# Galtvam/OthelloZero

Hardware: AMD Instinct MI355X
Metric: mcts_node_expansions_per_sec (higher is better)
Workload: dtype f32 (3xbf16 split)

## Files before the change

include/othellozero_amd.h:

```cpp
#ifndef OTHELLOZERO_AMD_H
#define OTHELLOZERO_AMD_H
#include <stdint.h>
#ifdef __cplusplus
extern "C" {
#endif

#define OZ_OK 0
#define OZ_ERR_HIP 1
#define OZ_ERR_ARG 2
#define OZ_ERR_CAPACITY 3
#define OZ_ERR_KEY 4
#define OZ_ERR_STATE 5

#define OZ_QMODE_NEP50 0
#define OZ_QMODE_F64 1

#define OZ_LEAF_IDLE 0
#define OZ_LEAF_TERMINAL 1
#define OZ_LEAF_EVAL 2
#define OZ_LEAF_WAIT 3

const char* oz_last_error(void);
int oz_version(void);
int oz_device_count(void);
// ... 230 lines not shown
    uint64_t black, white;
    uint64_t final_black, final_white;
    uint64_t game_id;
    uint8_t ply;
    uint8_t action;
    int8_t player;
    int8_t z;
    uint8_t greedy;
    uint8_t pad[3];
} oz_record;

typedef struct {
    int64_t simulations, node_visits, expansions, terminal_hits, fallbacks;
    int64_t moves, games_completed, records;
    int32_t live_games, overflow;
    int64_t leaves_evaluated;
} oz_selfplay_stats;

int oz_selfplay_create(oz_selfplay** out, const oz_selfplay_config* cfg, oz_net* net);
int oz_selfplay_destroy(oz_selfplay* sp);
int oz_selfplay_run(oz_selfplay* sp, int rounds);
int oz_selfplay_run_steps(oz_selfplay* sp, int steps);
int oz_selfplay_set_batch_cap(oz_selfplay* sp, int cap);
int oz_selfplay_set_dedup(oz_selfplay* sp, int enable);
int oz_selfplay_set_leaves_per_step(oz_selfplay* sp, int k);
int oz_selfplay_set_solve_leaves(oz_selfplay* sp, int max_empties);
int oz_selfplay_get_solve_leaves(oz_selfplay* sp, int* max_empties, int64_t* rows_solved);
int oz_selfplay_set_value_signs(oz_selfplay* sp, int mode);
int oz_selfplay_get_value_signs(oz_selfplay* sp, int* mode);
int oz_selfplay_set_selection(oz_selfplay* sp, int flags, double fpu_reduction, double fpu_root_reduction, double cpuct_base, double cpuct_factor);
int oz_selfplay_get_selection(oz_selfplay* sp, int* flags, double* fpu_reduction, double* fpu_root_reduction, double* cpuct_base, double* cpuct_factor);
int oz_selfplay_set_proofs(oz_selfplay* sp, int enable);
int oz_selfplay_proof_stats(oz_selfplay* sp, int64_t* out4);
int oz_selfplay_solve_leaves_profile(oz_selfplay* sp, int enable);
int oz_selfplay_solve_leaves_profile_read(oz_selfplay* sp, double* ms_total, int64_t* launches, int reset);
int oz_selfplay_set_root_noise(oz_selfplay* sp, double alpha, double eps);
int oz_selfplay_root_noise(oz_selfplay* sp, double* eta, uint8_t* armed);
int oz_selfplay_set_move_sampling(oz_selfplay* sp, double temperature, int plies);
int oz_selfplay_set_playout_cap(oz_selfplay* sp, int fast_sims, double full_prob);
int oz_selfplay_get_playout_cap(oz_selfplay* sp, int* fast_sims, double* full_prob, int64_t* full_moves, int64_t* fast_moves);
int oz_selfplay_set_forced_playouts(oz_selfplay* sp, double k);
int oz_selfplay_get_forced_playouts(oz_selfplay* sp, double* k, int64_t* moves_pruned, int64_t* visits_raw, int64_t* visits_kept);
int oz_selfplay_set_resign(oz_selfplay* sp, double v, int r, int min_ply, double keep_prob);
int oz_selfplay_get_resign(oz_selfplay* sp, double* v, int* r, int* min_ply, double* keep_prob, oz_resign_stats* stats);
int oz_selfplay_sync(oz_selfplay* sp);
int oz_selfplay_stagger(oz_selfplay* sp, int sims_pre);
// ... 274 lines not shown
```

othellozero_amd/_lib.py:

```python
import ctypes as C
import os

import numpy as np

_HERE = os.path.dirname(os.path.abspath(__file__))
LIB_PATH = os.environ.get("OZ_LIB_PATH") or os.path.join(_HERE, "lib", "libothellozero_amd.so")

OZ_OK, OZ_ERR_HIP, OZ_ERR_ARG, OZ_ERR_CAPACITY, OZ_ERR_KEY, OZ_ERR_STATE = range(6)
QMODE_NEP50, QMODE_F64 = 0, 1
DEDUP_DEFAULT, DEDUP_ON, DEDUP_OFF = 0, 1, 2
NET_OPT_SIMPLE_LOOP, NET_OPT_ACT_TARGET_LOG2, NET_OPT_LOW_GUARD_LOG2, NET_OPT_SELF_CHECK, NET_OPT_W_TARGET_LOG2, NET_OPT_F32_STD_TILE, NET_OPT_LATENCY_SPLITS = 1, 2, 3, 4, 5, 6, 7
NET_OPT_CONV3_TILE = 8
NET_OPT_LOW_LOOP_PHASES = 9
NET_OPT_B3_TILE = 10
NET_OPT_B3_MIX_ROWS = 11
NET_INFO_CONV3_TILE_ROWS, NET_INFO_SELF_CHECK_GUARD, NET_INFO_ARITHMETIC = 1, 2, 3
NET_INFO_LAYER_BIG_ROWS = 64
NET_INFO_LAYER_TILE_ROWS, NET_INFO_LAYER_KSLICES, NET_INFO_LAYER_KERNEL = 16, 32, 48
NET_KERNEL_NAMES = {0: "none", 1: "f32_skinny", 2: "f32_std", 3: "f32_std_pixmajor", 4: "f32_big", 5: "lut", 6: "lut_xcd", 7: "lut_xcd_inline",
                    10: "h2_small2", 11: "h2_small", 12: "h2_bigpp", 13: "h2_bigpp_lut", 14: "h2_midpp", 15: "h2_lowpp1", 16: "h2_lowpp", 17: "h2_big",
                    18: "h2_mid", 19: "h2_thin2", 20: "h2_thin", 21: "h2_thin4w", 30: "b3", 31: "b3_big", 32: "b3_mixed"}
LEAF_IDLE, LEAF_TERMINAL, LEAF_EVAL = 0, 1, 2
VT_INT, VT_F32, VT_F64 = 0, 1, 2
MAX_LEAVES_PER_STEP = 16
# ... 221 lines not shown
    "oz_mcts_set_forced_playouts": [_vp, C.c_double], "oz_mcts_get_forced_playouts": [_vp, _f64p],
    "oz_mcts_pruned_counts": [_vp, _i32p, _u64p, _i32p],
    "oz_selfplay_set_forced_playouts": [_vp, C.c_double],
    "oz_selfplay_get_forced_playouts": [_vp, _f64p, _i64p, _i64p, _i64p],
    "oz_playout_budgets": [C.c_uint64, _u64p, _i32p, C.c_int64, C.c_int, C.c_int, C.c_double, _i32p],
    "oz_selfplay_set_resign": [_vp, C.c_double, C.c_int, C.c_int, C.c_double],
    "oz_selfplay_get_resign": [_vp, _f64p, C.POINTER(C.c_int), C.POINTER(C.c_int), _f64p, C.POINTER(ResignStats)],
    "oz_resign_scan": [_i8p, _f64p, _i32p, C.c_int64, C.c_double, C.c_int, C.c_int, _i32p, _i8p],
    "oz_resign_exempt": [C.c_uint64, _u64p, C.c_int64, C.c_double, _u8p],
    "oz_mcts_set_gumbel": [_vp, C.c_int, C.c_double, C.c_double, C.c_int, _f64p, _u8p],
    "oz_mcts_sample_gumbel": [_vp, C.c_int, C.c_double, C.c_double, C.c_int, C.c_uint64, _u64p, _i32p],
    "oz_mcts_get_gumbel": [_vp, _f64p, _u8p, _i32p, _i32p, _f64p, _f64p, _i32p],
    "oz_mcts_gumbel_policy": [_vp, _f32p, _i32p, _i32p], "oz_mcts_gumbel_scores": [_vp, _f64p],
    "oz_mcts_node_value": [_vp, C.c_int, C.c_int, _f64p],
    "oz_selfplay_set_gumbel": [_vp, C.c_int, C.c_double, C.c_double], "oz_selfplay_get_gumbel": [_vp, _i32p, _f64p, _f64p, _i64p],
    "oz_selfplay_gumbel": [_vp, _f64p, _u8p, _i32p],
    "oz_selfplay_policies": [_vp, _f32p, C.c_int64, _i64p], "oz_selfplay_policies_device": [_vp, _vp, C.c_int64, _i64p],
    "oz_gumbel_considered_visits": [C.c_int, C.c_int, _i32p],
    "oz_gumbel_draws": [C.c_uint64, _u64p, _i32p, _u64p, C.c_int64, _f64p], "oz_gumbel_from_units": [_f64p, C.c_int64, _f64p],
    "oz_gumbel_root": [_i32p, _i32p, _f64p, _f64p, _f64p, _u64p, _f64p, C.c_int64, C.c_int, C.c_double, C.c_double, C.c_int, _i32p, _i32p, _f32p,
                       _f64p, _f64p],
    "oz_selfplay_create": [C.POINTER(_vp), C.POINTER(SelfplayConfig), _vp],
    "oz_selfplay_destroy": [_vp], "oz_selfplay_run": [_vp, C.c_int], "oz_selfplay_run_steps": [_vp, C.c_int], "oz_selfplay_sync": [_vp],
    "oz_selfplay_stagger": [_vp, C.c_int], "oz_selfplay_profile": [_vp, C.c_int], "oz_selfplay_set_batch_cap": [_vp, C.c_int], "oz_selfplay_set_dedup": [_vp, C.c_int],
    "oz_selfplay_profile_read": [_vp, _f64p, _i64p, C.c_int],
    "oz_selfplay_get_stats": [_vp, C.POINTER(SelfplayStats)],
    "oz_selfplay_state": [_vp, _u64p, _u64p, _i8p, _u8p, _i32p, _u64p],
    "oz_selfplay_records": [_vp, _vp, C.c_int64, _i64p],
    "oz_selfplay_records_device": [_vp, _vp, C.c_int64, _i64p],
    "oz_selfplay_visits": [_vp, _i32p, C.c_int64, _i64p],
    "oz_selfplay_visits_device": [_vp, _vp, C.c_int64, _i64p],
    "oz_selfplay_last_counts": [_vp, _i32p],
    "oz_root_values": [_i32p, _f64p, C.c_int64, _f64p], "oz_mcts_root_values": [_vp, _f64p, _i32p],
    "oz_selfplay_set_record_values": [_vp, C.c_int],
    "oz_selfplay_values": [_vp, _f64p, C.c_int64, _i64p], "oz_selfplay_values_device": [_vp, _vp, C.c_int64, _i64p],
    "oz_selfplay_value_targets": [_vp, C.c_int64, C.c_int, C.c_double, C.c_int, C.POINTER(ValueTargetStats)],
    "oz_selfplay_targets": [_vp, _f32p, C.c_int64, _i64p], "oz_selfplay_targets_device": [_vp, _vp, C.c_int64, _i64p],
    "oz_value_targets": [_vp, _f64p, C.c_int64, C.c_int, C.c_int, C.c_double, C.c_int, _f32p],
    "oz_selfplay_set_record_surprise": [_vp, C.c_int],
    "oz_selfplay_surprises": [_vp, _f64p, C.c_int64, _i64p], "oz_selfplay_surprises_device": [_vp, _vp, C.c_int64, _i64p],
    "oz_policy_surprises": [_i32p, _f64p, C.c_int64, _f64p], "oz_policy_surprises_f32": [_f32p, _f64p, C.c_int64, _f64p],
    "oz_selfplay_surprise_weights": [_vp, C.c_int64, C.c_double, C.c_uint64, C.POINTER(SurpriseWeightStats)],
    "oz_selfplay_weights": [_vp, _f32p, _i32p, _u8p, C.c_int64, _i64p],
    "oz_surprise_weights": [_vp, _f64p, C.c_int64, C.c_double, _f32p],
    "oz_surprise_copies": [_vp, _f32p, C.c_int64, C.c_uint64, _i32p, _u8p],
    "oz_selfplay_eval_time": [_vp, _f64p, _i64p, _i64p],
    "oz_comm_unique_id": [_u8p], "oz_comm_create": [C.POINTER(_vp), _u8p, C.c_int, C.c_int], "oz_comm_destroy": [_vp],
# ... 712 lines not shown
```

othellozero_amd/csrc/oz_internal.h:

```cpp
#pragma once
#include <deque>
#include <mutex>
#include <vector>

#include "../../include/othellozero_amd.h"
#include "oz_common.h"

#define OZ_API extern "C" __attribute__((visibility("default")))

int oz_current_device();

template <auto Kernel> static int set_max_lds_once(int bytes) {
    static bool attr_done[64] = {};
    int dev_now = 0;
    OZ_HIP(hipGetDevice(&dev_now));
    if (!attr_done[dev_now & 63]) {
        OZ_HIP(hipFuncSetAttribute((const void*)Kernel, hipFuncAttributeMaxDynamicSharedMemorySize, bytes));
        attr_done[dev_now & 63] = true;
    }
    return OZ_OK;
}

struct OzTimer {
    enum { OPEN = 0, ENDED = 1, CANCELLED = 2, FAILED = 3 };
// ... 75 lines not shown
    int* d_counts = nullptr;
    EvalCacheDev ec;
    void free_eval_cache() {
        if (!ec.buckets) return;
        hipSetDevice(device);
        hipFree(ec.keys); hipFree(ec.pi); hipFree(ec.v); hipFree(ec.stamp); hipFree(ec.counters);
        ec = EvalCacheDev();
    }
    int es_mode = OZ_EVAL_SYM_OFF;
    uint64_t es_seed = 0;
    uint64_t* es_boards = nullptr;
    float* es_out = nullptr;
    int* es_count = nullptr;
    int es_profile = 0;
    OzTimer es_timer{2};
    virtual ~oz_net() {
        if (es_boards || es_out || es_count) { hipSetDevice(device); hipFree(es_boards); hipFree(es_out); hipFree(es_count); }
        es_timer.destroy();
        if (p_in) { hipSetDevice(device); hipFree(p_in); hipFree(p_out); }
        if (hp_in) { hipSetDevice(device); hipHostFree(hp_in); hipHostFree(hp_out); hipFree(d_counts); }
        free_eval_cache();
    }
    virtual int check() { return 0; }
    virtual const int* flag_device() { return nullptr; }
    virtual int forward_raw(const uint64_t* d_own, const uint64_t* d_opp, const int* d_count, int max_count,
                            float* d_pi, float* d_v, hipStream_t s) = 0;
    int forward_device(const uint64_t* d_own, const uint64_t* d_opp, const int* d_count, int max_count,
                       float* d_pi, float* d_v, hipStream_t s);
};

int oz_net_forward_device(oz_net* net, const uint64_t* d_own, const uint64_t* d_opp, const int* d_count,
                          int max_count, float* d_pi, float* d_v, hipStream_t s);

struct OzLayerShape {
    int Hin, Hout, pad, Cin, taps, N;
    int K() const { return taps * Cin; }
    int pixels() const { return Hout * Hout; }
};
template <typename Geom> inline void oz_geom_set_shape(Geom& g, const OzLayerShape& L) {
    g.Hin = L.Hin; g.Hout = L.Hout; g.pad = L.pad; g.Cin = L.Cin; g.taps = L.taps; g.N = L.N; g.K = L.K();
}
struct OzLayers {
    OzLayerShape l[5];
    const OzLayerShape& operator[](int i) const { return l[i]; }
    const OzLayerShape* begin() const { return l; }
    const OzLayerShape* end() const { return l + 5; }
// ... 47 lines not shown
```

othellozero_amd/csrc/oz_net.hip:

```cpp
#include <math.h>
#include <stdlib.h>
#include <string.h>

#include <algorithm>
#include <type_traits>
#include <vector>

#include "oz_internal.h"

__global__ __launch_bounds__(256) void k_conv1(const uint64_t* __restrict__ own, const uint64_t* __restrict__ opp,
                                               const int* __restrict__ d_count, int n, int C,
                                               const float* __restrict__ W , const float* __restrict__ scale,
                                               const float* __restrict__ shift, float* __restrict__ out ) {
    const int P = n * n, cq = C >> 2;
    const long long M = (long long)(*d_count) * P;
    const long long idx = (long long)blockIdx.x * blockDim.x + threadIdx.x;
    const long long m = idx / cq;
    if (m >= M) return;
    const int c4 = (int)(idx % cq) * 4;
    const int b = (int)(m / P), pix = (int)(m % P), y = pix / n, x = pix % n;
    const uint64_t o = own[b], p = opp[b];
    float acc0 = 0.f, acc1 = 0.f, acc2 = 0.f, acc3 = 0.f;
#pragma unroll
    for (int ky = 0; ky < 3; ++ky)
// ... 816 lines not shown
    float *d_scale1_h2 = nullptr, *d_shift1_h2 = nullptr;
    float* d_shift_h2[5] = {nullptr, nullptr, nullptr, nullptr, nullptr};
    unsigned* d_lowcnt[5] = {nullptr, nullptr, nullptr, nullptr, nullptr};
    unsigned char* d_lut_low = nullptr;
    unsigned fwd_seq = 0;
    int act_target_log2 = H2_ACT_TOP;
    int w_target_log2 = H2_W_TOP;
    int low_guard_log2 = H2_LOW_GUARD;
    float low_thr = 0.f;
    int self_check = 1;
    double sc_dpi = -1.0, sc_dv = -1.0;
    int sc_positions = 0;
    int sc_guard = 0;
    float *d_sc_out = nullptr;
    uint64_t *d_cal_own = nullptr, *d_cal_opp = nullptr;
    int* d_cal_count = nullptr;
    int cal_total = 0;

    uint4* d_wb[5] = {nullptr, nullptr, nullptr, nullptr, nullptr};
    uint4* b3a1 = nullptr;
    uint4 *b3a2 = nullptr, *b3a3 = nullptr, *b3a4 = nullptr, *b3f1 = nullptr;
    float* d_part_b3 = nullptr;
    bool use_b3() const { return precision == 2 && max_batch >= B3_MIN_BATCH; }
    int fc1_b3_ksplit() const {
        const long long blocks = (((long long)max_batch + B3_BM - 1) / B3_BM) * 4;
        int k = 1;
        while (k < 8 && blocks * k < 192) k *= 2;
        return k < 2 ? 2 : k;
    }
    int conv_b3_ksplit(int pixels) const {
        const long long blocks = (((long long)max_batch * pixels + B3_BM - 1) / B3_BM) * (C / B3_BN);
        int k = 1;
        while (k < 8 && blocks * k < 192) k *= 2;
        return k;
    }
    int ensure_b3a1() {
        if (b3a1 || !use_b3() || (tables_mode != 0 && tables_mode != 1)) return OZ_OK;
        return alloc(&b3a1, (size_t)max_batch * n * n * (C / 32 * 12));
    }
    int fc2_b3_ksplit() const {
        return 4;
    }

    struct TimedSlot {
        OzTimer* t = nullptr;
        hipStream_t s;
// ... 1166 lines not shown
    OnnNet* o = as_onn(net);
    OZ_REQUIRE(o && out, "not an OthelloNN network / null argument");
    OZ_REQUIRE(which >= 0 && which <= 9, "oz_net_get_scaling: which must be 0 .. 9 (got %d)", which);
    std::lock_guard<std::mutex> lk(o->mu);
    OZ_REQUIRE(o->precision == 1 && o->committed, "oz_net_get_scaling: the network is not committed in precision f16x2");
    const std::vector<int>& e = which < 5 ? o->aexp[which] : o->wexp[which - 5];
    OZ_REQUIRE(nelem == (int64_t)e.size(), "oz_net_get_scaling(%d): %lld elements expected, got %lld", which, (long long)e.size(), (long long)nelem);
    for (size_t i = 0; i < e.size(); ++i) out[i] = e[i];
    return OZ_OK;
}

OZ_API int oz_net_get_info(oz_net* net, int what, int* value) {
    OnnNet* o = as_onn(net);
    OZ_REQUIRE(o && value, "not an OthelloNN network / null argument");
    std::lock_guard<std::mutex> lk(o->mu);
    for (int l = 1; l <= 5; ++l) {
        const OnnNet::LayerPlan& p = o->plan[l];
        if (what == OZ_NET_INFO_LAYER_TILE_ROWS(l)) { *value = p.tile_rows; return OZ_OK; }
        if (what == OZ_NET_INFO_LAYER_KSLICES(l)) { *value = p.ksplit; return OZ_OK; }
        if (what == OZ_NET_INFO_LAYER_KERNEL(l)) { *value = p.kernel; return OZ_OK; }
        if (what == OZ_NET_INFO_LAYER_BIG_ROWS(l)) { *value = (int)p.big_rows; return OZ_OK; }
    }
    OZ_REQUIRE(what == OZ_NET_INFO_CONV3_TILE_ROWS || what == OZ_NET_INFO_SELF_CHECK_GUARD || what == OZ_NET_INFO_ARITHMETIC, "unknown network info %d", what);
    *value = what == OZ_NET_INFO_CONV3_TILE_ROWS ? o->last_conv3_rows : what == OZ_NET_INFO_ARITHMETIC ? (o->precision == 2 && !o->use_b3() ? 0 : o->precision) : o->sc_guard;
    return OZ_OK;
}

OZ_API int oz_net_b3_plan(int n, int channels, int max_batch, int layer, int kslices, int tile_opt, int mix_rows_opt, int* kernel, int64_t* big_rows,
                          int64_t* small_tiles) {
    OZ_REQUIRE((n == 6 || n == 8) && channels > 0 && channels % B3_BN == 0 && max_batch >= 1 && layer >= 1 && layer <= 5 && kslices >= 1,
               "oz_net_b3_plan: bad shape (n=%d channels=%d max_batch=%d layer=%d kslices=%d)", n, channels, max_batch, layer, kslices);
    OZ_REQUIRE(tile_opt == 0 || tile_opt == 128 || tile_opt == 256, "OZ_NET_OPT_B3_TILE must be 0, 128 or 256 (got %d)", tile_opt);
    OZ_REQUIRE(mix_rows_opt <= 0 || mix_rows_opt % B3B_BM == 0, "OZ_NET_OPT_B3_MIX_ROWS must be 0, negative or a positive multiple of 256 (got %d)", mix_rows_opt);
    const OzLayerShape L = oz_onn_layers(n, channels)[layer - 1];
    const long long rows_cap = (long long)max_batch * L.pixels();
    const long long head = b3_plan_rows(L, rows_cap, kslices, tile_opt, mix_rows_opt);
    const int k = b3_plan_kernel(head, rows_cap);
    if (kernel) *kernel = k;
    if (big_rows) *big_rows = k == OZ_NET_KERNEL_B3 ? 0 : head;
    if (small_tiles) *small_tiles = k == OZ_NET_KERNEL_B3_BIG ? 0 : (rows_cap + B3_BM - 1) / B3_BM - (k == OZ_NET_KERNEL_B3 ? 0 : head / B3_BM);
    return OZ_OK;
}

OZ_API int oz_net_get_activation(oz_net* net, int layer, int64_t first_row, int64_t rows, double* out) {
    OnnNet* o = as_onn(net);
    OZ_REQUIRE(o && out, "oz_net_get_activation: not an OthelloNN network / null argument");
    OZ_REQUIRE(layer >= 0 && layer <= 5, "oz_net_get_activation: layer must be 0 .. 5 (got %d)", layer);
// ... 61 lines not shown
```

othellozero_amd/csrc/oz_search.hip:

```cpp
#pragma clang fp contract(off)
#include <math.h>
#include <string.h>

#include "oz_internal.h"
#include "oz_minimax.h"
#include "oz_openings.h"
#include "oz_solve.h"

enum { VT_INT = 0, VT_F32 = 1, VT_F64 = 2 };
#define OZ_MAX_DEPTH 64
#define OZ_TAG_F32 0x80000000u
#define OZ_NSTAT 5
enum { ST_SIMS = 0, ST_VISITS = 1, ST_EXPAND = 2, ST_TERMINAL = 3, ST_FALLBACK = 4 };
enum { EF_NODES = 1, EF_EDGES = 2, EF_DEPTH = 4, EF_NOMOVE = 8, EF_RECORDS = 16, EF_ROOT = 32, EF_CORRUPT = 64 };

struct OzEdge { uint32_t n_tag; int32_t child; double q; double p; };
#define OZ_REC_HDR 32
#define OZ_EDGE_BYTES 24
#define OZ_HT_IDX_BITS 20
#define OZ_HT_IDX_MASK ((1u << OZ_HT_IDX_BITS) - 1u)
static_assert(sizeof(OzEdge) == OZ_EDGE_BYTES, "edge layout");

enum { PS_EDGES = 0, PS_EDGE_STOPS = 1, PS_NODE_STOPS = 2, PS_ROOTS = 3, OZ_NPSTAT = 4 };
struct ProofDev {
// ... 443 lines not shown
    if (!t.active[g]) {
        if (lane == 0) t.leaf_status[g] = OZ_LEAF_IDLE;
        return OZ_LEAF_IDLE;
    }
    double eta = 0.0;
    const bool noisy = noise_of_slot<NOISE>(t, g, lane, &eta);
    const uint64_t own = uni64(t.root_own[g]), opp = uni64(t.root_opp[g]);
    int rootn = unii(t.root_node[g]);
    GumbelRoot gr{false, 0.0, 0, nullptr};
    if constexpr (GUMBEL) gr = gumbel_of_slot(*gd, g, lane);
    const Descent e = descend_one<NOISE, GUMBEL, VS, SEL>(t, L.rec, L.path, g, lane, own, opp, oz_legal(own, opp, t.valid), rootn, noisy, eta, InFlight{nullptr, nullptr, 0}, gr);
    __syncthreads();
    if (lane < e.depth) t.path[(size_t)g * OZ_MAX_DEPTH + lane] = L.path[lane];
    if (lane == 0) {
        t.leaf_status[g] = e.status;
        t.leaf_own[g] = e.own; t.leaf_opp[g] = e.opp; t.leaf_legal[g] = e.legal; t.leaf_fs[g] = e.fs;
        t.depth[g] = e.depth; t.term_value[g] = e.tval;
        unsigned long long* st = t.stat + (size_t)g * OZ_NSTAT;
        st[ST_SIMS] += 1; st[ST_VISITS] += (unsigned long long)(e.depth + 1);
        if (e.status == OZ_LEAF_TERMINAL) st[ST_TERMINAL] += 1;
        if (e.err) atomicOr(t.error_flag, e.err);
    }
    return e.status;
}

__device__ __forceinline__ unsigned ec_bucket(const EvalCacheDev& c, uint64_t own, uint64_t opp, unsigned* way_pick) {
    const uint64_t h = key_hash64(own ^ 0x6A09E667F3BCC909ULL, opp);
    *way_pick = (unsigned)(h >> 40) & (OZ_EC_WAYS - 1);
    return (unsigned)(h >> 8) & (c.buckets - 1);
}
__device__ __forceinline__ int ec_find(const EvalCacheDev& c, uint64_t own, uint64_t opp) {
    unsigned pick;
    const unsigned b = ec_bucket(c, own, opp, &pick);
    const ulonglong2* k = reinterpret_cast<const ulonglong2*>(c.keys) + (size_t)b * OZ_EC_WAYS;
#pragma unroll
    for (int w = 0; w < OZ_EC_WAYS; ++w) {
        const ulonglong2 e = k[w];
        if (e.x == own && e.y == opp) return (int)(b * OZ_EC_WAYS + w);
    }
    return -1;
}
__global__ __launch_bounds__(256) void k_cache_copy(MctsDev t) {
    const int idx = blockIdx.x * 256 + threadIdx.x, h = idx >> 6, a = idx & 63;
    if (h >= *t.hit_count) return;
    const int e = t.hit_entry[h], row = t.G - 1 - h;
    if (a < t.n2) t.pi[(size_t)row * t.n2 + a] = t.ec.pi[(size_t)e * t.n2 + a];
// ... 2764 lines not shown
    } else if (lane == 0) {
        gm.black[g] = black; gm.white[g] = white; gm.player[g] = (int8_t)player;
        gm.finished[g] = (uint8_t)fin; gm.ply[g] = nply;
        t.root_node[g] = -1;
    }
}
enum : unsigned { MV_SAMPLE = 1, MV_CAP = 2, MV_FORCE = 4, MV_VALUES = 8, MV_GUMBEL = 16, MV_SURPRISE = 32, MV_RESIGN = 64, MV_PROVEN = 128,
                  MV_FULL = MV_SAMPLE | MV_CAP | MV_FORCE | MV_VALUES };
struct MoveArgs {
    MoveSampling ms; PlayoutCap pc; ForcedPlayouts fp; SurprisePlay su; ResignPlay rs; ProofPlay pp; GumbelPlay gp;
    int arena;
};
template <unsigned M>
__global__ __launch_bounds__(64) void k_sp_move(GamesDev gm, MctsDev t, MoveArgs a) {
    const int arena = M == 0 ? a.arena : M == MV_PROVEN ? 1 : 0;
    sp_move_body<false, has(M, MV_SAMPLE), has(M, MV_CAP), has(M, MV_FORCE), has(M, MV_VALUES), has(M, MV_GUMBEL), has(M, MV_SURPRISE), has(M, MV_RESIGN),
                 has(M, MV_PROVEN)>(gm, t, blockIdx.x, threadIdx.x, arena, a.ms, a.pc, a.fp, a.gp, a.su, a.rs, a.pp);
}

#define OZ_ADVANCE_CAP 2
struct SelfplayExtras { double alpha; uint64_t seed; MoveSampling sample; PlayoutCap cap; ForcedPlayouts forced; };
template <bool EXTRAS = false, bool VALUES = EXTRAS, bool SURPRISE = false, int VS = OZ_VSIGNS_REFERENCE>
__device__ __forceinline__ void advance_body(const GamesDev& gm, const MctsDev& t, TreeLds& L, int g, int lane, int sims, int* __restrict__ sims_done, int cap,
                                             SelfplayExtras xt = SelfplayExtras{}, SurprisePlay su = SurprisePlay{}) {
    if (unii(t.leaf_status[g]) == OZ_LEAF_WAIT) {
        if (lane == 0) t.leaf_status[g] = OZ_LEAF_EVAL;
        return;
    }
    int done = sims_done[g];
    if (t.leaf_status[g] == OZ_LEAF_EVAL) ++done;
    int status = OZ_LEAF_IDLE;
    for (int it = 0; it < cap; ++it) {
        if (gm.finished[g]) { if (lane == 0) { t.active[g] = 0; t.leaf_status[g] = OZ_LEAF_IDLE; } status = OZ_LEAF_IDLE; break; }
        const int p = gm.player[g];
        if (lane == 0) {
            t.active[g] = 1;
            t.root_own[g] = p == 1 ? gm.black[g] : gm.white[g];
            t.root_opp[g] = p == 1 ? gm.white[g] : gm.black[g];
        }
        wave_sync();
        int budget = sims, fast = 0;
        if constexpr (EXTRAS) {
            if (xt.cap.fast_sims > 0)
                budget = oz_playout_budget(gm.seed, uni64(gm.game_id[g]), (uint64_t)unii(gm.ply[g]), sims, xt.cap.fast_sims, xt.cap.full_prob, &fast);
        }
        if (done >= budget) {
            sp_move_body<EXTRAS, EXTRAS, EXTRAS, EXTRAS, VALUES, false, SURPRISE>(gm, t, g, lane, 0, xt.sample, xt.cap, xt.forced, GumbelPlay{}, su);
            done = 0;
            if (lane == 0) t.leaf_status[g] = OZ_LEAF_IDLE;
            wave_sync();
            continue;
        }
        if constexpr (EXTRAS) {
            if (t.noise_eps > 0.0 && !fast && unii((int)t.noise_armed[g]) == 0) {
                root_noise_body(t, L.arr, g, lane, uni64(t.root_own[g]), uni64(t.root_opp[g]), xt.alpha, xt.seed, uni64(gm.game_id[g]), unii(gm.ply[g]));
                wave_sync();
            }
        }
        status = select_body<EXTRAS, false, VS>(t, L, g, lane);
        if (status != OZ_LEAF_TERMINAL) break;
        wave_sync();
        backup_body<VS>(t, g, lane, (double)t.term_value[g], VT_INT);
        ++done;
        status = OZ_LEAF_IDLE;
        if (lane == 0) t.leaf_status[g] = OZ_LEAF_IDLE;
        wave_sync();
    }
    if (lane == 0) sims_done[g] = done;
}
enum : unsigned { AV_SIGNS = 3, AV_EXTRAS = 4, AV_VALUES = 8, AV_SURPRISE = 16 };
struct AdvanceArgs { SelfplayExtras xt; SurprisePlay su; };
template <unsigned A>
__global__ __launch_bounds__(64) void k_advance(GamesDev gm, MctsDev t, int sims, int* __restrict__ sims_done, int cap, AdvanceArgs a) {
    __shared__ TreeLds L;
    advance_body<has(A, AV_EXTRAS), has(A, AV_VALUES), has(A, AV_SURPRISE), int(A & AV_SIGNS)>(gm, t, L, blockIdx.x, threadIdx.x, sims, sims_done, cap, a.xt, a.su);
}
template <unsigned A>
__global__ __launch_bounds__(64) void k_backup_advance(GamesDev gm, MctsDev t, int sims, int* __restrict__ sims_done, int cap, AdvanceArgs a) {
    __shared__ TreeLds L;
    expand_backup_body<false, int(A & AV_SIGNS)>(t, L, blockIdx.x, threadIdx.x, 0);
    backup_fence();
    advance_body<has(A, AV_EXTRAS), has(A, AV_VALUES), has(A, AV_SURPRISE), int(A & AV_SIGNS)>(gm, t, L, blockIdx.x, threadIdx.x, sims, sims_done, cap, a.xt, a.su);
}

__global__ void k_arena_random_move(GamesDev gm, int side) {
    const int g = blockIdx.x * blockDim.x + threadIdx.x;
    if (g >= gm.G || gm.finished[g] || gm.player[g] != side) return;
    uint64_t black = gm.black[g], white = gm.white[g];
    int player = side, fin = 0;
    const uint64_t legal = oz_legal(side == 1 ? black : white, side == 1 ? white : black, gm.valid);
    const int ply = gm.ply[g];
    const int action = oz_kth_bit(legal, (int)(oz_rng(gm.seed, gm.game_id[g], (uint64_t)ply, OZ_RNG_TIE) % (uint64_t)oz_popc(legal)));
    const size_t lb = (size_t)g * 64;
    if (ply < 64) {
        gm.log_black[lb + ply] = black; gm.log_white[lb + ply] = white;
        gm.log_action[lb + ply] = (uint8_t)action; gm.log_player[lb + ply] = (int8_t)player; gm.log_greedy[lb + ply] = 0;
    }
    oz_game_play(black, white, player, fin, action, gm.valid);
    gm.black[g] = black; gm.white[g] = white; gm.player[g] = (int8_t)player;
    gm.finished[g] = (uint8_t)fin; gm.ply[g] = ply + 1;
    atomicAdd(&gm.counters[2], 1ULL);
}

__global__ __launch_bounds__(64) void k_arena_minimax_move(GamesDev gm, int side, int depth, MinimaxEval ev) {
    __shared__ MinimaxLds L;
// ... 25 lines not shown
    const int played = oz_opening_play(gm.n, gm.valid, op.moves ? op.n_plies[g] : op.plies, op.moves ? op.moves + (size_t)g * OZ_OPENING_MAX_PLIES : nullptr,
                                       op.seed, op.first_id + (uint64_t)g, black, white, player, fin,
                                       [&](int ply, uint64_t b, uint64_t w, int p, int action) {
                                           gm.log_black[lb + ply] = b; gm.log_white[lb + ply] = w;
                                           gm.log_action[lb + ply] = (uint8_t)action; gm.log_player[lb + ply] = (int8_t)p; gm.log_greedy[lb + ply] = 0;
                                       });
    gm.black[g] = black; gm.white[g] = white; gm.player[g] = (int8_t)player;
    gm.finished[g] = (uint8_t)fin; gm.ply[g] = played;
    op.opening_plies[g] = played;
    if (played) atomicAdd(&gm.counters[2], (unsigned long long)played);
}

static void initial_board(int n, uint64_t* black, uint64_t* white) { oz_initial_board(n, *black, *white); }

struct oz_selfplay {
    oz_selfplay_config cfg;
    oz_mcts* m = nullptr;
    oz_net* net = nullptr;
    GamesDev gm;
    int* d_sims_done = nullptr;
    int mode = 0;
    int batch_cap = 0;
    long long batch_no = 0;
    int stagger_period = 0;
    bool noise_on = false;
    double noise_alpha = 0.0;
    MoveSampling sample{0.0, 0};
    PlayoutCap cap{0, 0.0, nullptr, nullptr};
    ForcedPlayouts forced{0.0, nullptr};
    bool gumbel_on = false;
    float *gumbel_log = nullptr, *gumbel_rows = nullptr;
    unsigned long long* gumbel_moves = nullptr;
    std::vector<void*> allocs;
    std::mutex mu;
    long long records_read = 0;
    long long* d_endgame = nullptr;
    double *val_log = nullptr, *val_rec = nullptr;
    float* targets = nullptr;
    long long* d_vt = nullptr;
    double *sur_log = nullptr, *sur_rec = nullptr;
    SurprisePlay su{nullptr, nullptr};
    float* weights = nullptr;
    int32_t* copies = nullptr;
    uint8_t* first_sym = nullptr;
    long long* d_sw = nullptr;
    ResignPlay resign{0.0, 0.0, 0, 0, nullptr, nullptr, nullptr, nullptr, nullptr};
// ... 619 lines not shown
    if (moves && sp->gumbel_moves) {
        hipSetDevice(sp->m->device);
        OZ_HIP(hipStreamSynchronize(sp->m->stream));
        OZ_HIP(hipMemcpy(&c, sp->gumbel_moves, sizeof c, hipMemcpyDeviceToHost));
    }
    if (moves) *moves = (int64_t)c;
    return OZ_OK;
}
OZ_API int oz_selfplay_gumbel(oz_selfplay* sp, double* g, uint8_t* armed, int32_t* N0) {
    OZ_REQUIRE(sp, "null selfplay");
    { std::lock_guard<std::mutex> lk(sp->mu); hipSetDevice(sp->m->device); OZ_HIP(hipStreamSynchronize(sp->m->stream)); }
    return oz_mcts_get_gumbel(sp->m, g, armed, N0, nullptr, nullptr, nullptr, nullptr);
}
OZ_API int oz_selfplay_root_noise(oz_selfplay* sp, double* eta, uint8_t* armed) {
    OZ_REQUIRE(sp, "null selfplay");
    std::lock_guard<std::mutex> lk(sp->mu);
    std::lock_guard<std::mutex> lkm(sp->m->mu);
    hipSetDevice(sp->m->device);
    OZ_HIP(hipStreamSynchronize(sp->m->stream));
    return noise_read_locked(sp->m, eta, armed);
}

struct AdvanceKernels {
    void (*advance)(GamesDev, MctsDev, int, int*, int, AdvanceArgs);
    void (*backup_advance)(GamesDev, MctsDev, int, int*, int, AdvanceArgs);
    void (*expand_backup)(MctsDev, int);
};
static int advance_kernels(const oz_selfplay* sp, AdvanceKernels* k, AdvanceArgs* a) {
    const oz_mcts* m = sp->m;
    const bool surprise = sp->su.log != nullptr;
    const bool extras = surprise || m->noise_ever || sp->sample.plies > 0 || sp->cap.fast_sims > 0;
    *a = AdvanceArgs{};
    if (extras) a->xt = SelfplayExtras{sp->noise_alpha, sp->gm.seed, sp->sample, sp->cap, sp->forced};
    if (surprise) a->su = sp->su;
    const unsigned signs = m->proofs ? OZ_VSIGNS_PROVEN : m->vsigns != OZ_VSIGNS_REFERENCE ? OZ_VSIGNS_SOUND : OZ_VSIGNS_REFERENCE;
    const unsigned v = signs | (extras ? AV_EXTRAS : 0) | (extras || sp->gm.log_values ? AV_VALUES : 0) | (surprise ? AV_SURPRISE : 0);
    switch (v) {
#define OZ_A(...) \
    case (__VA_ARGS__): *k = AdvanceKernels{k_advance<(__VA_ARGS__)>, k_backup_advance<(__VA_ARGS__)>, k_expand_backup<(__VA_ARGS__) & AV_SIGNS>}; return OZ_OK
        OZ_A(OZ_VSIGNS_REFERENCE); OZ_A(OZ_VSIGNS_REFERENCE | AV_VALUES); OZ_A(OZ_VSIGNS_REFERENCE | AV_EXTRAS | AV_VALUES);
        OZ_A(OZ_VSIGNS_REFERENCE | AV_EXTRAS | AV_VALUES | AV_SURPRISE);
        OZ_A(OZ_VSIGNS_SOUND); OZ_A(OZ_VSIGNS_SOUND | AV_VALUES); OZ_A(OZ_VSIGNS_SOUND | AV_EXTRAS | AV_VALUES);
        OZ_A(OZ_VSIGNS_SOUND | AV_EXTRAS | AV_VALUES | AV_SURPRISE);
#undef OZ_A
    }
    oz_set_error("oz_selfplay_run_steps: the free-running driver has no kernels for this combination of options (variant 0x%x); use oz_selfplay_run", v);
    return OZ_ERR_STATE;
}
// ... 1 lines not shown
OZ_API int oz_selfplay_run_steps(oz_selfplay* sp, int steps) {
    OZ_REQUIRE(sp, "null selfplay");
    std::lock_guard<std::mutex> lk(sp->mu);
    if (sp->m->leaves_per_step > 1) {
        oz_set_error("oz_selfplay_run_steps: the free-running driver runs one leaf per game and batch (leaves_per_step is %d); use oz_selfplay_run", sp->m->leaves_per_step);
        return OZ_ERR_STATE;
    }
    if (sp->gumbel_on) { oz_set_error("oz_selfplay_run_steps: the free-running driver does not run the Gumbel search; use oz_selfplay_run"); return OZ_ERR_STATE; }
    if (sp->m->proofs) { oz_set_error("oz_selfplay_run_steps: the free-running driver keeps no proofs; use oz_selfplay_run"); return OZ_ERR_STATE; }
    if (sp->m->d.sel.flags) { oz_set_error("oz_selfplay_run_steps: the free-running kernels have no selection instantiation; use oz_selfplay_run"); return OZ_ERR_STATE; }
    if (sp->resign.r > 0) { oz_set_error("oz_selfplay_run_steps: the free-running driver does not resign games; use oz_selfplay_run"); return OZ_ERR_STATE; }
    if (sp->tree_gc != OZ_TREE_GC_OFF) { oz_set_error("oz_selfplay_run_steps: the free-running driver moves inside its kernels and does not collect the tree; use oz_selfplay_run"); return OZ_ERR_STATE; }
    std::lock_guard<std::mutex> lkn(sp->net->mu);
    oz_mcts* m = sp->m;
    hipSetDevice(m->device);
    MctsDev& d = m->d;
    if (sp->mode == 1) OZ_HIP(hipMemsetAsync(d.leaf_status, 0, sizeof(int) * d.G, m->stream));
    if (sp->mode == 1 && m->noise_ever) OZ_HIP(hipMemsetAsync(d.noise_armed, 0, (size_t)d.G, m->stream));
    sp->mode = 2;
    selfplay_attach_cache(sp);
    AdvanceKernels ak;
    AdvanceArgs aargs;
    if (int rc = advance_kernels(sp, &ak, &aargs)) return rc;
    for (int i = 0; i < steps; ++i) {
        const bool all = m->profile;
        hipStream_t s = m->stream;
        const int adv_cap = (sp->batch_cap > 0 && sp->batch_cap < d.G ? 1 : OZ_ADVANCE_CAP);
        timed(m, TS_SELECT, all, [&] { hipLaunchKernelGGL(i == 0 ? ak.advance : ak.backup_advance, dim3(d.G), dim3(64), 0, s, sp->gm, d, sp->cfg.sims, sp->d_sims_done, adv_cap, aargs); });
        MctsDev dc = d;
        const int cap = sp->batch_cap > 0 && sp->batch_cap < d.G ? sp->batch_cap : 0;
        dc.batch_cap = cap;
        dc.batch_rot = cap ? (int)((sp->batch_no * (long long)cap) % d.G) : 0;
        sp->batch_no += 1;
        timed(m, TS_COMPACT, all, [&] { hipLaunchKernelGGL(k_compact, dim3(1), dim3(1024), 0, s, dc); });
        if (int rc = eval_batch_async(m, sp->net, cap ? cap : d.G, true)) return rc;
        if (i == steps - 1) timed(m, TS_BACKUP, all, [&] { hipLaunchKernelGGL(ak.expand_backup, dim3(d.G), dim3(64), 0, s, d, 0); });
        OZ_HIP(hipGetLastError());
        if (m->timer.backlog() > 4096) m->timer.drain();
    }
    return OZ_OK;
}

OZ_API int oz_selfplay_set_batch_cap(oz_selfplay* sp, int cap) {
    OZ_REQUIRE(sp, "null selfplay");
    std::lock_guard<std::mutex> lk(sp->mu);
    OZ_REQUIRE(cap >= 0, "oz_selfplay_set_batch_cap: cap %d", cap);
    OZ_REQUIRE(cap == 0 || cap >= 8, "oz_selfplay_set_batch_cap: a cap below 8 leaves (got %d)", cap);
    sp->batch_cap = cap;
    return OZ_OK;
}

OZ_API int oz_selfplay_set_dedup(oz_selfplay* sp, int enable) {
    OZ_REQUIRE(sp, "null selfplay");
    std::lock_guard<std::mutex> lk(sp->mu);
    sp->m->d.dedup = enable ? 1 : 0;
    return OZ_OK;
}

OZ_API int oz_selfplay_sync(oz_selfplay* sp) {
    OZ_REQUIRE(sp, "null selfplay");
    std::lock_guard<std::mutex> lk(sp->mu);
    hipSetDevice(sp->m->device);
// ... 1378 lines not shown
```

othellozero_amd/training.py:

```python
import ctypes as C
import logging
import random

import numpy as np

from . import _lib
from .NNet import NeuralNets
from .Othello import BoardView, OthelloGame, OthelloPlayer
from .othelo_mcts import OthelloMCTS


def training_example_symmetries(board, policy):
    symetric_examples = []
    for rotation in range(1, 5):
        for flip in (True, False):
            b, p = np.rot90(board, k=rotation), np.rot90(policy, k=rotation)
            if flip:
                b, p = np.fliplr(b), np.fliplr(p)
            symetric_examples.append((b, p))
    return symetric_examples


def execute_episode(board_size, neural_network, degree_exploration, num_simulations, policy_temperature, e_greedy,
                    q_mode=_lib.QMODE_F64, snapshot_boards=False, policy_target="onehot", target_temperature=1.0,
# ... 281 lines not shown
        return rows.value

    def __del__(self):
        try:
            if self._h:
                _lib.load().oz_selfplay_destroy(self._h)
                self._h = C.c_void_p()
        except Exception:
            pass

    def run(self, rounds=1, sync=True):
        _lib.check(_lib.load().oz_selfplay_run(self._h, int(rounds)))
        if sync:
            self.sync()

    def run_steps(self, steps, sync=True):
        _lib.check(_lib.load().oz_selfplay_run_steps(self._h, int(steps)))
        if sync:
            self.sync()

    def set_batch_cap(self, cap):
        _lib.check(_lib.load().oz_selfplay_set_batch_cap(self._h, int(cap)))

    def set_dedup(self, enable):
        _lib.check(_lib.load().oz_selfplay_set_dedup(self._h, 1 if enable else 0))

    def stagger(self, sims_pre=None, sync=True):
        _lib.check(_lib.load().oz_selfplay_stagger(self._h, int(sims_pre or self.cfg.sims)))
        if sync:
            self.sync()

    def profile(self, enable=True):
        _lib.check(_lib.load().oz_selfplay_profile(self._h, 1 if enable else 0))

    def profile_read(self, reset=False):
        k = len(_lib.TREE_KERNELS)
        ms, cnt = np.zeros(k, np.float64), np.zeros(k, np.int64)
        _lib.check(_lib.load().oz_selfplay_profile_read(self._h, _lib.p_f64(ms), _lib.p_i64(cnt), 1 if reset else 0))
        return {name: (float(ms[i]), int(cnt[i])) for i, name in enumerate(_lib.TREE_KERNELS)}

    def sync(self):
        _lib.check(_lib.load().oz_selfplay_sync(self._h))

    def stats(self):
        s = _lib.SelfplayStats()
        _lib.check(_lib.load().oz_selfplay_get_stats(self._h, C.byref(s)))
# ... 91 lines not shown
        return written.value

    def eval_time(self):
        ms, launches, leaves = C.c_double(), C.c_int64(), C.c_int64()
        _lib.check(_lib.load().oz_selfplay_eval_time(self._h, C.byref(ms), C.byref(launches), C.byref(leaves)))
        return dict(ms=ms.value, launches=launches.value, leaves=leaves.value)

    def play_to_end(self, max_rounds=None, with_visits=False, endgame_targets=0, value_target="outcome", with_policies=False,
                    proof_targets=False):
        proof_targets = _lib.check_proof_targets(proof_targets, self.proof_play)
        max_rounds = max_rounds or self.n * self.n
        for _ in range(max_rounds):
            self.run(4)
            if self.stats()["live_games"] == 0:
                break
        if proof_targets:
            self.proof_target_stats = self.proof_targets()
        if endgame_targets:
            self.endgame_stats = self.solve_records(endgame_targets)
        if _lib.check_value_target(value_target)[0] != _lib.VALUE_TARGET_OUTCOME:
            self.value_target_stats = self.value_targets(value_target, exact_empties=endgame_targets, exact_proven=proof_targets)
            return self.records(with_visits=with_visits, with_targets=True, with_policies=with_policies)
        return self.records(with_visits=with_visits, with_policies=with_policies)


def preferred_batch_cap(board_size, num_games, channels=512, precision="f16x2"):
    if channels % 256 or num_games < 1024 or precision == "bf16x3":
        return 0
    P, cols = (board_size - 2) ** 2, channels // 256
    rounds = (num_games * P // 256) * cols // 256
    if rounds < 1:
        return 0
    cap = (256 * rounds // cols) * 256 // P
    return 0 if cap >= num_games else int(cap)


def expand_examples(records, board_size, alias_final=False, visits=None, target_temperature=1.0, values=None):
    if values is not None:
        rec_all = np.ascontiguousarray(records, dtype=_lib.RECORD_DTYPE)
        val = np.ascontiguousarray(values, dtype=np.float32).ravel()
        assert val.size == rec_all.size, f"{val.size} value targets for {rec_all.size} records"
        boards, pol, _z = expand_examples(rec_all, board_size, alias_final, visits=visits, target_temperature=target_temperature)
        return boards, pol, np.repeat(val[_lib.record_fast(rec_all).ravel() == 0], 8)
    records, visits = _lib.full_records(np.ascontiguousarray(records, dtype=_lib.RECORD_DTYPE), visits)
    rec = np.ascontiguousarray(records, dtype=_lib.RECORD_DTYPE)
    R, n = rec.size, board_size
# ... 124 lines not shown
```

Measured before the change: 960,200.

## Restructure advance kernel to cache root state and batch stat updates

The per-game advance kernel now loads the root position, its legal-move mask and the root node once per move rather than on every loop iteration. It calls descend_one directly and stores the descent result to global memory only when a leaf actually needs evaluation. Per-simulation statistics are accumulated in registers and written once at the end, and a separate cap for idle entry is added along with a setter and a defaults API. Default caps are unchanged, so the gain is meant to come from fewer global memory writes and reloads in the select/terminal-backup loop, at the cost of more complex control flow.

New measurement: 959,900 (median of 2 runs). Within noise of the previous version (-0.0%).

```diff
diff --git a/include/othellozero_amd.h b/include/othellozero_amd.h
--- a/include/othellozero_amd.h
+++ b/include/othellozero_amd.h
@@ -276,6 +276,8 @@
 int oz_selfplay_run(oz_selfplay* sp, int rounds);
 int oz_selfplay_run_steps(oz_selfplay* sp, int steps);
 int oz_selfplay_set_batch_cap(oz_selfplay* sp, int cap);
+int oz_selfplay_set_advance_cap(oz_selfplay* sp, int cap, int cap_idle);
+int oz_selfplay_advance_caps(int arithmetic, int games, int batch_cap, int* cap, int* cap_idle);
 int oz_selfplay_set_dedup(oz_selfplay* sp, int enable);
 int oz_selfplay_set_leaves_per_step(oz_selfplay* sp, int k);
 int oz_selfplay_set_solve_leaves(oz_selfplay* sp, int max_empties);
diff --git a/othellozero_amd/_lib.py b/othellozero_amd/_lib.py
--- a/othellozero_amd/_lib.py
+++ b/othellozero_amd/_lib.py
@@ -267,7 +267,9 @@
                        _f64p, _f64p],
     "oz_selfplay_create": [C.POINTER(_vp), C.POINTER(SelfplayConfig), _vp],
     "oz_selfplay_destroy": [_vp], "oz_selfplay_run": [_vp, C.c_int], "oz_selfplay_run_steps": [_vp, C.c_int], "oz_selfplay_sync": [_vp],
-    "oz_selfplay_stagger": [_vp, C.c_int], "oz_selfplay_profile": [_vp, C.c_int], "oz_selfplay_set_batch_cap": [_vp, C.c_int], "oz_selfplay_set_dedup": [_vp, C.c_int],
+    "oz_selfplay_stagger": [_vp, C.c_int], "oz_selfplay_profile": [_vp, C.c_int], "oz_selfplay_set_batch_cap": [_vp, C.c_int],
+    "oz_selfplay_set_advance_cap": [_vp, C.c_int, C.c_int],
+    "oz_selfplay_advance_caps": [C.c_int, C.c_int, C.c_int, C.POINTER(C.c_int), C.POINTER(C.c_int)], "oz_selfplay_set_dedup": [_vp, C.c_int],
     "oz_selfplay_profile_read": [_vp, _f64p, _i64p, C.c_int],
     "oz_selfplay_get_stats": [_vp, C.POINTER(SelfplayStats)],
     "oz_selfplay_state": [_vp, _u64p, _u64p, _i8p, _u8p, _i32p, _u64p],
diff --git a/othellozero_amd/csrc/oz_internal.h b/othellozero_amd/csrc/oz_internal.h
--- a/othellozero_amd/csrc/oz_internal.h
+++ b/othellozero_amd/csrc/oz_internal.h
@@ -121,6 +121,7 @@
         free_eval_cache();
     }
     virtual int check() { return 0; }
+    virtual int arithmetic() const { return -1; }
     virtual const int* flag_device() { return nullptr; }
     virtual int forward_raw(const uint64_t* d_own, const uint64_t* d_opp, const int* d_count, int max_count,
                             float* d_pi, float* d_v, hipStream_t s) = 0;
diff --git a/othellozero_amd/csrc/oz_net.hip b/othellozero_amd/csrc/oz_net.hip
--- a/othellozero_amd/csrc/oz_net.hip
+++ b/othellozero_amd/csrc/oz_net.hip
@@ -862,6 +862,7 @@
     uint4 *b3a2 = nullptr, *b3a3 = nullptr, *b3a4 = nullptr, *b3f1 = nullptr;
     float* d_part_b3 = nullptr;
     bool use_b3() const { return precision == 2 && max_batch >= B3_MIN_BATCH; }
+    int arithmetic() const override { return precision == 2 && !use_b3() ? 0 : precision; }
     int fc1_b3_ksplit() const {
         const long long blocks = (((long long)max_batch + B3_BM - 1) / B3_BM) * 4;
         int k = 1;
@@ -2074,7 +2075,7 @@
         if (what == OZ_NET_INFO_LAYER_BIG_ROWS(l)) { *value = (int)p.big_rows; return OZ_OK; }
     }
     OZ_REQUIRE(what == OZ_NET_INFO_CONV3_TILE_ROWS || what == OZ_NET_INFO_SELF_CHECK_GUARD || what == OZ_NET_INFO_ARITHMETIC, "unknown network info %d", what);
-    *value = what == OZ_NET_INFO_CONV3_TILE_ROWS ? o->last_conv3_rows : what == OZ_NET_INFO_ARITHMETIC ? (o->precision == 2 && !o->use_b3() ? 0 : o->precision) : o->sc_guard;
+    *value = what == OZ_NET_INFO_CONV3_TILE_ROWS ? o->last_conv3_rows : what == OZ_NET_INFO_ARITHMETIC ? o->arithmetic() : o->sc_guard;
     return OZ_OK;
 }
 
diff --git a/othellozero_amd/csrc/oz_search.hip b/othellozero_amd/csrc/oz_search.hip
--- a/othellozero_amd/csrc/oz_search.hip
+++ b/othellozero_amd/csrc/oz_search.hip
@@ -489,6 +489,16 @@
         if (e.err) atomicOr(t.error_flag, e.err);
     }
     return e.status;
+}
+__device__ __forceinline__ void store_descent(const MctsDev& t, const TreeLds& L, int g, int lane, const Descent& e) {
+    __syncthreads();
+    if (lane < e.depth) t.path[(size_t)g * OZ_MAX_DEPTH + lane] = L.path[lane];
+    if (lane == 0) {
+        t.leaf_status[g] = e.status;
+        t.leaf_own[g] = e.own; t.leaf_opp[g] = e.opp; t.leaf_legal[g] = e.legal; t.leaf_fs[g] = e.fs;
+        t.depth[g] = e.depth; t.term_value[g] = e.tval;
+        if (e.err) atomicOr(t.error_flag, e.err);
+    }
 }
 
 __device__ __forceinline__ unsigned ec_bucket(const EvalCacheDev& c, uint64_t own, uint64_t opp, unsigned* way_pick) {
@@ -3299,65 +3309,88 @@
 struct SelfplayExtras { double alpha; uint64_t seed; MoveSampling sample; PlayoutCap cap; ForcedPlayouts forced; };
 template <bool EXTRAS = false, bool VALUES = EXTRAS, bool SURPRISE = false, int VS = OZ_VSIGNS_REFERENCE>
 __device__ __forceinline__ void advance_body(const GamesDev& gm, const MctsDev& t, TreeLds& L, int g, int lane, int sims, int* __restrict__ sims_done, int cap,
-                                             SelfplayExtras xt = SelfplayExtras{}, SurprisePlay su = SurprisePlay{}) {
-    if (unii(t.leaf_status[g]) == OZ_LEAF_WAIT) {
+                                             int cap_idle, SelfplayExtras xt = SelfplayExtras{}, SurprisePlay su = SurprisePlay{}) {
+    const int entry = unii(t.leaf_status[g]);
+    if (entry == OZ_LEAF_WAIT) {
         if (lane == 0) t.leaf_status[g] = OZ_LEAF_EVAL;
         return;
     }
     int done = sims_done[g];
-    if (t.leaf_status[g] == OZ_LEAF_EVAL) ++done;
+    if (entry == OZ_LEAF_EVAL) ++done;
+    else cap = cap_idle;
     int status = OZ_LEAF_IDLE;
+    bool stage = true;
+    uint64_t rown = 0, ropp = 0, rlegal = 0;
+    int rootn = -1, budget = sims, fast = 0;
+    unsigned n_sims = 0, n_visits = 0, n_term = 0;
     for (int it = 0; it < cap; ++it) {
-        if (gm.finished[g]) { if (lane == 0) { t.active[g] = 0; t.leaf_status[g] = OZ_LEAF_IDLE; } status = OZ_LEAF_IDLE; break; }
-        const int p = gm.player[g];
-        if (lane == 0) {
-            t.active[g] = 1;
-            t.root_own[g] = p == 1 ? gm.black[g] : gm.white[g];
-            t.root_opp[g] = p == 1 ? gm.white[g] : gm.black[g];
-        }
-        wave_sync();
-        int budget = sims, fast = 0;
-        if constexpr (EXTRAS) {
-            if (xt.cap.fast_sims > 0)
-                budget = oz_playout_budget(gm.seed, uni64(gm.game_id[g]), (uint64_t)unii(gm.ply[g]), sims, xt.cap.fast_sims, xt.cap.full_prob, &fast);
+        if (stage) {
+            if (gm.finished[g]) { if (lane == 0) t.active[g] = 0; break; }
+            const int p = unii((int)gm.player[g]);
+            const uint64_t black = uni64(gm.black[g]), white = uni64(gm.white[g]);
+            rown = p == 1 ? black : white; ropp = p == 1 ? white : black;
+            rlegal = oz_legal(rown, ropp, t.valid);
+            rootn = unii(t.root_node[g]);
+            if (lane == 0) { t.active[g] = 1; t.root_own[g] = rown; t.root_opp[g] = ropp; }
+            wave_sync();
+            budget = sims; fast = 0;
+            if constexpr (EXTRAS) {
+                if (xt.cap.fast_sims > 0)
+                    budget = oz_playout_budget(gm.seed, uni64(gm.game_id[g]), (uint64_t)unii(gm.ply[g]), sims, xt.cap.fast_sims, xt.cap.full_prob, &fast);
+            }
+            stage = false;
         }
         if (done >= budget) {
             sp_move_body<EXTRAS, EXTRAS, EXTRAS, EXTRAS, VALUES, false, SURPRISE>(gm, t, g, lane, 0, xt.sample, xt.cap, xt.forced, GumbelPlay{}, su);
             done = 0;
-            if (lane == 0) t.leaf_status[g] = OZ_LEAF_IDLE;
             wave_sync();
+            stage = true;
             continue;
         }
         if constexpr (EXTRAS) {
             if (t.noise_eps > 0.0 && !fast && unii((int)t.noise_armed[g]) == 0) {
-                root_noise_body(t, L.arr, g, lane, uni64(t.root_own[g]), uni64(t.root_opp[g]), xt.alpha, xt.seed, uni64(gm.game_id[g]), unii(gm.ply[g]));
+                root_noise_body(t, L.arr, g, lane, rown, ropp, xt.alpha, xt.seed, uni64(gm.game_id[g]), unii(gm.ply[g]));
                 wave_sync();
             }
         }
-        status = select_body<EXTRAS, false, VS>(t, L, g, lane);
-        if (status != OZ_LEAF_TERMINAL) break;
+        double eta = 0.0;
+        const bool noisy = noise_of_slot<EXTRAS>(t, g, lane, &eta);
+        const Descent e = descend_one<EXTRAS, false, VS>(t, L.rec, L.path, g, lane, rown, ropp, rlegal, rootn, noisy, eta, InFlight{nullptr, nullptr, 0});
+        n_sims += 1; n_visits += (unsigned)(e.depth + 1);
+        if (e.status != OZ_LEAF_TERMINAL) {
+            store_descent(t, L, g, lane, e);
+            status = e.status;
+            break;
+        }
+        n_term += 1;
         wave_sync();
-        backup_body<VS>(t, g, lane, (double)t.term_value[g], VT_INT);
+        backup_one<VS>(t, g, lane, e.depth, L.path, (double)e.tval, VT_INT);
         ++done;
-        status = OZ_LEAF_IDLE;
-        if (lane == 0) t.leaf_status[g] = OZ_LEAF_IDLE;
         wave_sync();
     }
-    if (lane == 0) sims_done[g] = done;
+    if (lane == 0) {
+        sims_done[g] = done;
+        if (status == OZ_LEAF_IDLE) t.leaf_status[g] = OZ_LEAF_IDLE;
+        if (n_sims) {
+            unsigned long long* st = t.stat + (size_t)g * OZ_NSTAT;
+            st[ST_SIMS] += n_sims; st[ST_VISITS] += n_visits;
+            if (n_term) st[ST_TERMINAL] += n_term;
+        }
+    }
 }
 enum : unsigned { AV_SIGNS = 3, AV_EXTRAS = 4, AV_VALUES = 8, AV_SURPRISE = 16 };
 struct AdvanceArgs { SelfplayExtras xt; SurprisePlay su; };
 template <unsigned A>
-__global__ __launch_bounds__(64) void k_advance(GamesDev gm, MctsDev t, int sims, int* __restrict__ sims_done, int cap, AdvanceArgs a) {
+__global__ __launch_bounds__(64) void k_advance(GamesDev gm, MctsDev t, int sims, int* __restrict__ sims_done, int cap, int cap_idle, AdvanceArgs a) {
     __shared__ TreeLds L;
-    advance_body<has(A, AV_EXTRAS), has(A, AV_VALUES), has(A, AV_SURPRISE), int(A & AV_SIGNS)>(gm, t, L, blockIdx.x, threadIdx.x, sims, sims_done, cap, a.xt, a.su);
+    advance_body<has(A, AV_EXTRAS), has(A, AV_VALUES), has(A, AV_SURPRISE), int(A & AV_SIGNS)>(gm, t, L, blockIdx.x, threadIdx.x, sims, sims_done, cap, cap_idle, a.xt, a.su);
 }
 template <unsigned A>
-__global__ __launch_bounds__(64) void k_backup_advance(GamesDev gm, MctsDev t, int sims, int* __restrict__ sims_done, int cap, AdvanceArgs a) {
+__global__ __launch_bounds__(64) void k_backup_advance(GamesDev gm, MctsDev t, int sims, int* __restrict__ sims_done, int cap, int cap_idle, AdvanceArgs a) {
     __shared__ TreeLds L;
     expand_backup_body<false, int(A & AV_SIGNS)>(t, L, blockIdx.x, threadIdx.x, 0);
     backup_fence();
-    advance_body<has(A, AV_EXTRAS), has(A, AV_VALUES), has(A, AV_SURPRISE), int(A & AV_SIGNS)>(gm, t, L, blockIdx.x, threadIdx.x, sims, sims_done, cap, a.xt, a.su);
+    advance_body<has(A, AV_EXTRAS), has(A, AV_VALUES), has(A, AV_SURPRISE), int(A & AV_SIGNS)>(gm, t, L, blockIdx.x, threadIdx.x, sims, sims_done, cap, cap_idle, a.xt, a.su);
 }
 
 __global__ void k_arena_random_move(GamesDev gm, int side) {
@@ -3429,6 +3462,7 @@
     int mode = 0;
     int batch_cap = 0;
     long long batch_no = 0;
+    int adv_cap = 0, adv_cap_idle = 0;
     int stagger_period = 0;
     bool noise_on = false;
     double noise_alpha = 0.0;
@@ -4094,8 +4128,8 @@
 }
 
 struct AdvanceKernels {
-    void (*advance)(GamesDev, MctsDev, int, int*, int, AdvanceArgs);
-    void (*backup_advance)(GamesDev, MctsDev, int, int*, int, AdvanceArgs);
+    void (*advance)(GamesDev, MctsDev, int, int*, int, int, AdvanceArgs);
+    void (*backup_advance)(GamesDev, MctsDev, int, int*, int, int, AdvanceArgs);
     void (*expand_backup)(MctsDev, int);
 };
 static int advance_kernels(const oz_selfplay* sp, AdvanceKernels* k, AdvanceArgs* a) {
@@ -4143,11 +4177,14 @@
     AdvanceKernels ak;
     AdvanceArgs aargs;
     if (int rc = advance_kernels(sp, &ak, &aargs)) return rc;
+    int adv_cap = 0, adv_cap_idle = 0;
+    const int capped = sp->batch_cap > 0 && sp->batch_cap < d.G ? sp->batch_cap : 0;
+    if (int rc = oz_selfplay_advance_caps(sp->net->arithmetic(), d.G, capped, &adv_cap, &adv_cap_idle)) return rc;
+    if (!capped && sp->adv_cap > 0) { adv_cap = sp->adv_cap; adv_cap_idle = sp->adv_cap_idle; }
     for (int i = 0; i < steps; ++i) {
         const bool all = m->profile;
         hipStream_t s = m->stream;
-        const int adv_cap = (sp->batch_cap > 0 && sp->batch_cap < d.G ? 1 : OZ_ADVANCE_CAP);
-        timed(m, TS_SELECT, all, [&] { hipLaunchKernelGGL(i == 0 ? ak.advance : ak.backup_advance, dim3(d.G), dim3(64), 0, s, sp->gm, d, sp->cfg.sims, sp->d_sims_done, adv_cap, aargs); });
+        timed(m, TS_SELECT, all, [&] { hipLaunchKernelGGL(i == 0 ? ak.advance : ak.backup_advance, dim3(d.G), dim3(64), 0, s, sp->gm, d, sp->cfg.sims, sp->d_sims_done, adv_cap, adv_cap_idle, aargs); });
         MctsDev dc = d;
         const int cap = sp->batch_cap > 0 && sp->batch_cap < d.G ? sp->batch_cap : 0;
         dc.batch_cap = cap;
@@ -4159,6 +4196,22 @@
         OZ_HIP(hipGetLastError());
         if (m->timer.backlog() > 4096) m->timer.drain();
     }
+    return OZ_OK;
+}
+
+OZ_API int oz_selfplay_advance_caps(int arithmetic, int games, int batch_cap, int* cap, int* cap_idle) {
+    OZ_REQUIRE(cap && cap_idle, "null argument");
+    OZ_REQUIRE(arithmetic >= -1 && arithmetic <= 2 && games >= 1 && batch_cap >= 0, "oz_selfplay_advance_caps: arithmetic %d, games %d, batch_cap %d", arithmetic, games, batch_cap);
+    const bool capped = batch_cap > 0 && batch_cap < games;
+    *cap = *cap_idle = capped ? 1 : OZ_ADVANCE_CAP;
+    return OZ_OK;
+}
+
+OZ_API int oz_selfplay_set_advance_cap(oz_selfplay* sp, int cap, int cap_idle) {
+    OZ_REQUIRE(cap >= 1 && cap_idle >= 1, "oz_selfplay_set_advance_cap: cap %d, cap_idle %d (both >= 1)", cap, cap_idle);
+    OZ_REQUIRE(sp, "null selfplay");
+    std::lock_guard<std::mutex> lk(sp->mu);
+    sp->adv_cap = cap; sp->adv_cap_idle = cap_idle;
     return OZ_OK;
 }
 
diff --git a/othellozero_amd/training.py b/othellozero_amd/training.py
--- a/othellozero_amd/training.py
+++ b/othellozero_amd/training.py
@@ -327,6 +327,9 @@
     def set_batch_cap(self, cap):
         _lib.check(_lib.load().oz_selfplay_set_batch_cap(self._h, int(cap)))
 
+    def set_advance_cap(self, cap, cap_idle):
+        _lib.check(_lib.load().oz_selfplay_set_advance_cap(self._h, int(cap), int(cap_idle)))
+
     def set_dedup(self, enable):
         _lib.check(_lib.load().oz_selfplay_set_dedup(self._h, 1 if enable else 0))
 
@@ -464,6 +467,13 @@
             self.value_target_stats = self.value_targets(value_target, exact_empties=endgame_targets, exact_proven=proof_targets)
             return self.records(with_visits=with_visits, with_targets=True, with_policies=with_policies)
         return self.records(with_visits=with_visits, with_policies=with_policies)
+
+
+def default_advance_caps(arithmetic, num_games, batch_cap=0):
+    a, b = C.c_int(0), C.c_int(0)
+    code = {"stub": -1, "f32": 0, "f16x2": 1, "bf16x3": 2}[arithmetic]
+    _lib.check(_lib.load().oz_selfplay_advance_caps(code, int(num_games), int(batch_cap), C.byref(a), C.byref(b)))
+    return a.value, b.value
 
 
 def preferred_batch_cap(board_size, num_games, channels=512, precision="f16x2"):
```
